# AaronZ345/StyleSinger

Hardware: AMD Instinct MI355X
Metric: mel-frames/sec (end-to-end infer incl. vocoder) (higher is better)
Workload: dtype f32; 1 GPU; c2: batch=8x8.0s utterances per GPU (T=1500 frames, Tp=28, Tr=1500), 100 mel + 2x100 f0 diffusion steps + HiFi-GAN-NSF, exact fp32 MFMA; global_batch=8, frames_per_utterance=1500, parallelism=dp1, diffusion_loops=hipGraph replay, hipgraph_captures=6, frame_bucket=64, mfma_precision=fp32, step_overlap=3 HIP streams: consecutive batches run concurrently

## Files before the change

stylesinger_amd/csrc/wino44_conv.hip:

```cpp
#include "common.h"
#include "device_prims.h"
#include "../../include/stylesinger_hip.h"
#include <type_traits>

namespace {

using namespace ss_dev;

constexpr int BK = 32;
constexpr int LD = BK;
constexpr int BQ = 64;
constexpr int NC = 7;
constexpr int NR = 7;

template <int D>
__device__ __forceinline__ int frame_of_quad(int q) {
  if constexpr (D == 1) return 4 * q;
  else return (q / D) * (4 * D) + (q % D);
}

template <int D, bool LRELU, int BN>
__global__ __launch_bounds__(BN * 4, BN == 64 ? 2 : 1) void wino44_conv_kernel(const ss_conv_gemm_args a, int q_tiles_per_item, int q_tiles,
                                                                               int n_tiles, int groups, int lo_rows) {
  static_assert(BN == 64 || BN == 32, "column tile of 64 or 32");
  constexpr int NT = BN * 4;
  constexpr int RP = NT / 8;
  constexpr int AP = BQ / RP;
  constexpr int BP = BN / RP;
  extern __shared__ __attribute__((aligned(16))) float smem[];
  float* As = smem;
  float* Bs = smem + 2 * BQ * LD;

  const int id = blockIdx.x;
  const int grp = id / (8 * n_tiles);
  const int rem = id % (8 * n_tiles);
  const int qt = grp * 8 + (rem & 7);
  const int nt = rem >> 3;
  if (qt >= q_tiles) return;
  const int b = __builtin_amdgcn_readfirstlane(qt / q_tiles_per_item);
  const int q0 = __builtin_amdgcn_readfirstlane((qt % q_tiles_per_item) * BQ);
  const int n0 = nt * BN;

  const int tid = threadIdx.x, lane = tid & 63, wave = tid >> 6;
  const int wm = BN == 64 ? wave >> 1 : wave, wn = BN == 64 ? wave & 1 : 0;
  const int l31 = lane & 31, lh = lane >> 5;

  const int len = ss_uniform_len(a.lens, b, a.T);
  const int kchunks = a.Kp / BK;
  const int ldw = groups * NC * a.Kp;

  const __amdgpu_buffer_rsrc_t rsrc_a = __builtin_amdgcn_make_buffer_rsrc(
      uniform_ptr(a.A + (int64_t)b * a.a_batch_stride), 0, __builtin_amdgcn_readfirstlane(len * a.lda * 4), 0x00020000);
  const __amdgpu_buffer_rsrc_t rsrc_w =
      __builtin_amdgcn_make_buffer_rsrc(uniform_ptr(a.W), 0, __builtin_amdgcn_readfirstlane(a.Np * ldw * 4), 0x00020000);

  const int st_c4 = tid & 7;
  const int st_row = tid >> 3;
  int roff[AP];
#pragma unroll
  for (int i = 0; i < AP; ++i) roff[i] = ((frame_of_quad<D>(q0 + st_row + i * RP) - lo_rows) * a.lda + st_c4 * 4) * 4;
  const int row_step = D * a.lda * 4;
  const int group_step = 4 * row_step;
  int w_voff[BP];
#pragma unroll
  for (int i = 0; i < BP; ++i) w_voff[i] = ((n0 + st_row + i * RP) * ldw + st_c4 * 4) * 4;

  using Yes = std::true_type;
  using No = std::false_type;
  u32x4 rr[AP][NR], rb[BP];
  auto load_rows = [&](int ci0b, auto ends) {
    ci0b = __builtin_amdgcn_readfirstlane(ci0b);
#pragma unroll
    for (int i = 0; i < AP; ++i)
#pragma unroll
      for (int r = 0; r < NR; ++r)
        if ((r == 0 || r == NR - 1) == decltype(ends)::value) rr[i][r] = __builtin_amdgcn_raw_buffer_load_b128(rsrc_a, roff[i] + r * row_step, ci0b, 0);
  };
  auto load_b = [&](int cb) {
    cb = __builtin_amdgcn_readfirstlane(cb);
#pragma unroll
    for (int i = 0; i < BP; ++i) rb[i] = __builtin_amdgcn_raw_buffer_load_b128(rsrc_w, w_voff[i], cb, 0);
  };
  const float slope = a.a_lrelu;
  auto act_rows = [&]() {
    if constexpr (LRELU) {
#pragma unroll
      for (int i = 0; i < AP; ++i)
#pragma unroll
        for (int r = 0; r < NR; ++r) {
          const f32x4 v = __builtin_bit_cast(f32x4, rr[i][r]);
          const f32x4 sv = v * slope;
          f32x4 o;
          o.x = ss_lrelu_max(v.x, sv.x);
          o.y = ss_lrelu_max(v.y, sv.y);
          o.z = ss_lrelu_max(v.z, sv.z);
          o.w = ss_lrelu_max(v.w, sv.w);
          rr[i][r] = __builtin_bit_cast(u32x4, o);
        }
    }
  };
  int a_wr[AP];
#pragma unroll
  for (int i = 0; i < AP; ++i) a_wr[i] = lds_slot(st_row + i * RP, st_c4);
  float4 tU[AP], tV[AP], tW[AP];
  auto store_a = [&](float* Ad, auto ptag) {
    constexpr int P = decltype(ptag)::value;
#pragma unroll
    for (int i = 0; i < AP; ++i) {
      auto R = [&](int q) { return __builtin_bit_cast(float4, rr[i][q]); };
      float4 v;
      if constexpr (P == 0) {
        tU[i] = vfma(4.f, R(1), vfma(-5.f, R(3), R(5)));
        tV[i] = vfma(4.f, R(0), vfma(-5.f, R(2), R(4)));
        tW[i] = vfma(4.f, R(2), vfma(-5.f, R(4), R(6)));
        v = tU[i];
      } else if constexpr (P == 1) {
        v = vfma(-0.5f, tU[i], tW[i]);
      } else if constexpr (P == 2) {
        v = vfma(-0.5f, tV[i], tU[i]);
      } else if constexpr (P == 3) {
        tV[i] = vfma(2.f, R(1), vfma(-4.f, R(2), vfma(-0.5f, R(3), R(4))));
        tU[i] = vfma(2.f, R(2), vfma(-4.f, R(3), vfma(-0.5f, R(4), R(5))));
        v = vadd(tU[i], tV[i]);
      } else if constexpr (P == 4) {
        v = vsub(tU[i], tV[i]);
      } else if constexpr (P == 5) {
        tV[i] = vfma(0.5f, R(1), vfma(-0.5f, R(3), vsub(R(4), R(2))));
        tU[i] = vfma(0.5f, R(2), vfma(-0.5f, R(4), vsub(R(5), R(3))));
        v = vfma(2.f, tV[i], tU[i]);
      } else {
        v = vfma(-2.f, tV[i], tU[i]);
      }
      *reinterpret_cast<float4*>(Ad + a_wr[i]) = v;
    }
  };
  auto store_b = [&](float* Bd) {
#pragma unroll
    for (int i = 0; i < BP; ++i)
      *reinterpret_cast<float4*>(Bd + lds_slot(st_row + i * RP, st_c4)) = __builtin_bit_cast(float4, rb[i]);
  };

  f32x16 acc[NC];
#pragma unroll
  for (int j = 0; j < NC; ++j)
#pragma unroll
    for (int r = 0; r < 16; ++r) acc[j][r] = 0.f;

  constexpr int ORD[NC] = {5, 6, 0, 1, 2, 3, 4};
  const int kb = a.Kp * 4;
  const int cs = BK * 4;
  const int steps = groups * kchunks;

  const int swz = (l31 >> 1) & 7;
  const int a_row = (wm * 32 + l31) * LD;
  const int b_row = (wn * 32 + l31) * LD;
  auto read_frags = [&](const float* Ac, const float* Bc, int q, float4& af, float4& bf) {
    const int so = ((2 * q + lh) ^ swz) << 2;
    af = *reinterpret_cast<const float4*>(Ac + a_row + so);
    bf = *reinterpret_cast<const float4*>(Bc + b_row + so);
  };
  auto mfma4 = [&](f32x16& c, const float4& af, const float4& bf) {
    c = __builtin_amdgcn_mfma_f32_32x32x2f32(af.x, bf.x, c, 0, 0, 0);
    c = __builtin_amdgcn_mfma_f32_32x32x2f32(af.y, bf.y, c, 0, 0, 0);
    c = __builtin_amdgcn_mfma_f32_32x32x2f32(af.z, bf.z, c, 0, 0, 0);
    c = __builtin_amdgcn_mfma_f32_32x32x2f32(af.w, bf.w, c, 0, 0, 0);
  };
  auto chunk = [&](auto etag, auto ptag, auto stage_tag, auto fetch_b_tag, auto fetch_rows_tag, int wb, int rows_cb, bool new_group) {
    constexpr int P = decltype(ptag)::value;
    constexpr int CUR = (decltype(etag)::value + P) & 1;
    constexpr int PN = (P + 1) % NC;
    const float* Ac = As + CUR * BQ * LD;
    const float* Bc = Bs + CUR * BN * LD;
    float4 af0, af1, bf0, bf1;
    read_frags(Ac, Bc, 0, af0, bf0);
    read_frags(Ac, Bc, 1, af1, bf1);
    __builtin_amdgcn_sched_barrier(0);
    mfma4(acc[ORD[P]], af0, bf0);
    read_frags(Ac, Bc, 2, af0, bf0);
    __builtin_amdgcn_sched_barrier(0);
    mfma4(acc[ORD[P]], af1, bf1);
    read_frags(Ac, Bc, 3, af1, bf1);
    __builtin_amdgcn_sched_barrier(0);
    if constexpr (decltype(stage_tag)::value) {
      if constexpr (PN == 0) act_rows();
      store_a(As + (CUR ^ 1) * BQ * LD, std::integral_constant<int, PN>{});
      store_b(Bs + (CUR ^ 1) * BN * LD);
    }
    __builtin_amdgcn_sched_barrier(0);
    if constexpr (decltype(fetch_b_tag)::value) load_b(wb);
    if constexpr (decltype(fetch_rows_tag)::value) {
      if constexpr (P == 4) {
        if (new_group) {
#pragma unroll
          for (int i = 0; i < AP; ++i) roff[i] += group_step;
        }
        load_rows(rows_cb, No{});
      } else {
        load_rows(rows_cb, Yes{});
      }
    }
    __builtin_amdgcn_sched_barrier(0);
    mfma4(acc[ORD[P]], af0, bf0);
    mfma4(acc[ORD[P]], af1, bf1);
    __syncthreads();
  };
  using P0 = std::integral_constant<int, 0>;
  using P1 = std::integral_constant<int, 1>;
  using P2 = std::integral_constant<int, 2>;
  using P3 = std::integral_constant<int, 3>;
  using P4 = std::integral_constant<int, 4>;
  using P5 = std::integral_constant<int, 5>;
  using P6 = std::integral_constant<int, 6>;

  int g = 0, k = 0;
  auto step = [&](auto etag) {
    const bool wrap = k + 1 == kchunks;
    const int gn = wrap ? g + 1 : g, kn = wrap ? 0 : k + 1;
    const int wcur = g * NC * kb + k * cs, wnext = gn * NC * kb + kn * cs;
    chunk(etag, P0{}, Yes{}, Yes{}, No{}, wcur + ORD[2] * kb, 0, false);
    chunk(etag, P1{}, Yes{}, Yes{}, No{}, wcur + ORD[3] * kb, 0, false);
    chunk(etag, P2{}, Yes{}, Yes{}, No{}, wcur + ORD[4] * kb, 0, false);
    chunk(etag, P3{}, Yes{}, Yes{}, No{}, wcur + ORD[5] * kb, 0, false);
    chunk(etag, P4{}, Yes{}, Yes{}, Yes{}, wcur + ORD[6] * kb, kn * cs, wrap);
    chunk(etag, P5{}, Yes{}, Yes{}, Yes{}, wnext + ORD[0] * kb, kn * cs, false);
    chunk(etag, P6{}, Yes{}, Yes{}, No{}, wnext + ORD[1] * kb, 0, false);
    g = gn;
    k = kn;
  };
  using E0 = std::integral_constant<int, 0>;
  using E1 = std::integral_constant<int, 1>;

  load_rows(0, No{});
  load_rows(0, Yes{});
  load_b(ORD[0] * kb);
  act_rows();
  store_a(As, P0{});
  store_b(Bs);
  load_b(ORD[1] * kb);
  __syncthreads();

  auto last_step = [&](auto etag) {
    const int wcur = g * NC * kb + k * cs;
    chunk(etag, P0{}, Yes{}, Yes{}, No{}, wcur + ORD[2] * kb, 0, false);
    chunk(etag, P1{}, Yes{}, Yes{}, No{}, wcur + ORD[3] * kb, 0, false);
    chunk(etag, P2{}, Yes{}, Yes{}, No{}, wcur + ORD[4] * kb, 0, false);
    chunk(etag, P3{}, Yes{}, Yes{}, No{}, wcur + ORD[5] * kb, 0, false);
    chunk(etag, P4{}, Yes{}, Yes{}, No{}, wcur + ORD[6] * kb, 0, false);
    chunk(etag, P5{}, Yes{}, No{}, No{}, 0, 0, false);
    chunk(etag, P6{}, No{}, No{}, No{}, 0, 0, false);
  };
  if constexpr (BN == 64) {
    for (int s = 0; s + 2 < steps; s += 2) {
      step(E0{});
      step(E1{});
    }
    step(E0{});
    last_step(E1{});
  } else {
    int left = steps;
    for (; left > 2; left -= 2) {
      step(E0{});
      step(E1{});
    }
    if (left == 2) {
      step(E0{});
      last_step(E1{});
    } else {
      last_step(E0{});
    }
  }

  const int col = n0 + wn * 32 + l31;
  const bool col_ok = col < a.N;
  const int oob = col_ok ? 0 : (int)0x80000000;
  const __amdgpu_buffer_rsrc_t rsrc_c = __builtin_amdgcn_make_buffer_rsrc(
      uniform_ptr(a.C + (int64_t)b * a.c_batch_stride), 0, __builtin_amdgcn_readfirstlane((int)((int64_t)a.T * a.ldc * 4)), 0x00020000);
  const __amdgpu_buffer_rsrc_t rsrc_r = __builtin_amdgcn_make_buffer_rsrc(
      uniform_ptr(a.R ? const_cast<float*>(a.R) + (int64_t)b * a.r_batch_stride : a.C), 0,
      __builtin_amdgcn_readfirstlane(a.R ? (int)((int64_t)a.T * a.ldr * 4) : 0), 0x00020000);
  const __amdgpu_buffer_rsrc_t rsrc_p = __builtin_amdgcn_make_buffer_rsrc(
      uniform_ptr(a.C + (int64_t)b * a.c_batch_stride), 0, __builtin_amdgcn_readfirstlane(a.accumulate ? (int)((int64_t)a.T * a.ldc * 4) : 0),
      0x00020000);
  const float bs = (a.bias && col_ok) ? a.bias[col] : 0.f;
  const int row_lim = a.mask_rows ? (len < a.T ? len : a.T) : a.T;
  const int ldc4 = a.ldc * 4, ldr4 = a.ldr * 4;
  const int qbase = q0 + wm * 32 + 4 * lh;
  const bool lrelu_out = a.act == SS_ACT_LRELU_;
#pragma unroll
  for (int rb4 = 0; rb4 < 4; ++rb4) {
    float rv[4][4], pv[4][4];
    int tq[4];
#pragma unroll
    for (int e = 0; e < 4; ++e) {
      tq[e] = frame_of_quad<D>(qbase + e + 8 * rb4);
#pragma unroll
      for (int o = 0; o < 4; ++o) {
        const int t = tq[e] + o * D;
        rv[e][o] = __builtin_bit_cast(float, __builtin_amdgcn_raw_buffer_load_b32(rsrc_r, t * ldr4 + (col * 4 + oob), 0, 0));
        pv[e][o] = __builtin_bit_cast(float, __builtin_amdgcn_raw_buffer_load_b32(rsrc_p, t * ldc4 + (col * 4 + oob), 0, 0));
      }
    }
#pragma unroll
    for (int e = 0; e < 4; ++e) {
      const int r = e + 4 * rb4;
      const float s12 = acc[1][r] + acc[2][r], d12 = acc[1][r] - acc[2][r];
      const float s34 = acc[3][r] + acc[4][r], d34 = acc[3][r] - acc[4][r];
      const float m5 = acc[5][r];
      float z[4];
      z[0] = (acc[0][r] + s12) + (s34 + m5);
      z[1] = fmaf(0.5f, m5, fmaf(2.0f, d34, d12));
      z[2] = fmaf(0.25f, m5, fmaf(4.0f, s34, s12));
      z[3] = fmaf(0.125f, m5, fmaf(8.0f, d34, d12)) + acc[6][r];
#pragma unroll
      for (int o = 0; o < 4; ++o) {
        const int t = tq[e] + o * D;
        float v = (z[o] + bs) * a.pre_scale;
        if (lrelu_out) v = ss_lrelu(v, a.act_slope);
        v = (v + rv[e][o]) * a.post_scale + pv[e][o];
        if (t >= row_lim) v = 0.f;
        __builtin_amdgcn_raw_buffer_store_b32(__builtin_bit_cast(unsigned, v), rsrc_c, t * ldc4 + (col * 4 + oob), 0, 0);
      }
    }
  }
}

template <int D, int BN>
void launch_conv(const ss_conv_gemm_args& a, int k, hipStream_t stream) {
  const int quads_per_item = ss_cdiv(a.T, 4 * D) * D;
  const int q_tiles_per_item = ss_cdiv(quads_per_item, BQ);
  const int q_tiles = q_tiles_per_item * a.B;
  const int n_tiles = a.Np / BN;
  const int grid = ss_cdiv(q_tiles, 8) * 8 * n_tiles;
  const size_t lds = (size_t)2 * (BQ + BN) * LD * sizeof(float);
  const int groups = (k + 3) / 4, lo = (k - 1) / 2 * D;
  auto go = [&](auto kernel) { hipLaunchKernelGGL(kernel, dim3(grid), dim3(BN * 4), lds, stream, a, q_tiles_per_item, q_tiles, n_tiles, groups, lo); };
  if (a.a_lrelu != 1.0f) go(wino44_conv_kernel<D, true, BN>);
  else go(wino44_conv_kernel<D, false, BN>);
}

template <int D>
void launch_conv(const ss_conv_gemm_args& a, int k, hipStream_t stream) {
  if (a.Np % 64 == 0) launch_conv<D, 64>(a, k, stream);
  else launch_conv<D, 32>(a, k, stream);
}

}

extern "C" int ss_wino44_conv_ok(int C, int k, int dilation) {
  const bool fewer = k >= 1 && k <= 11 && (k & 1) && ((k + 3) / 4) * 7 < ((k + 2) / 3) * 6;
  return fewer && C > 0 && C % 32 == 0 && (dilation == 1 || dilation == 3 || dilation == 5) ? 1 : 0;
}

extern "C" int ss_wino44_conv(const ss_conv_gemm_args* args, int k, int dilation, void* stream) {
  SS_CHECK_ARG(args != nullptr, "ss_wino44_conv: null args");
  const ss_conv_gemm_args& a = *args;
  SS_CHECK_ARG(a.A && a.W && a.C, "ss_wino44_conv: null A/W/C");
  SS_CHECK_ARG(a.Cin == a.N && ss_wino44_conv_ok(a.Cin, k, dilation), "ss_wino44_conv: Cin=%d == N=%d (multiple of 32), k=%d (7|11), dilation=%d (1|3|5)",
               a.Cin, a.N, k, dilation);
  SS_CHECK_ARG(a.Kp == a.Cin && a.Np == a.N && (a.lda & 3) == 0 && a.lda >= a.Cin, "ss_wino44_conv: Kp == Cin, Np == N, lda a multiple of 4");
  SS_CHECK_ARG(a.epi == SS_EPI_STORE && (a.act == SS_ACT_NONE_ || a.act == SS_ACT_LRELU_) && !a.a_bias && a.a_scale == 1.0f && !a.mfma_bf16 &&
                   a.group_size == 0,
               "ss_wino44_conv: STORE epilogue, act none|lrelu, no input bias/scale, fp32, one weight set");
  SS_CHECK_ARG(a.a_lrelu > 0.0f && a.a_lrelu <= 1.0f, "ss_wino44_conv: input leaky-relu slope %g must be in (0, 1]", (double)a.a_lrelu);
  SS_CHECK_ARG(((int64_t)a.T + 1024) * a.lda * 4 < (1ll << 31) && (int64_t)a.T * a.ldc * 4 < (1ll << 31) &&
                   (!a.R || (int64_t)a.T * a.ldr * 4 < (1ll << 31)) && (int64_t)a.Np * ((k + 3) / 4) * NC * a.Kp * 4 < (1ll << 31),
               "ss_wino44_conv: item too large for 32-bit offsets");
  if (dilation == 1) launch_conv<1>(a, k, (hipStream_t)stream);
  else if (dilation == 3) launch_conv<3>(a, k, (hipStream_t)stream);
  else launch_conv<5>(a, k, (hipStream_t)stream);
  SS_CHECK_LAUNCH("ss_wino44_conv");
  return SS_OK;
}
```

Measured before the change: 44220 mel-frames/s.

## Reuse Winograd input transforms across tap groups via halo rows in LDS

The Winograd F(4,4)-style conv kernel now stages the transformed input tile once, with extra halo rows (AR=80 rows, four transform slots), and reads shifted rows for each tap group instead of reloading and retransforming the input per group. The number of groups becomes a compile-time template parameter (2 for k=7, 3 for k=11), and the per-chunk schedule is fully unrolled over groups × transform positions, with input fetches spread across sub-steps. This is meant to cut global loads and transform ALU work, at the cost of much more LDS per block and larger, more complex unrolled code that may affect occupancy.

```diff
diff --git a/stylesinger_amd/csrc/wino44_conv.hip b/stylesinger_amd/csrc/wino44_conv.hip
--- a/stylesinger_amd/csrc/wino44_conv.hip
+++ b/stylesinger_amd/csrc/wino44_conv.hip
@@ -12,6 +12,14 @@
 constexpr int BQ = 64;
 constexpr int NC = 7;
 constexpr int NR = 7;
+constexpr int AR = 80;
+constexpr int NA = 4;
+constexpr int SLOT[7] = {0, 1, 2, 0, 1, 2, 3};
+
+__device__ __forceinline__ int formed_here(int x) {
+  asm volatile("" : "+v"(x));
+  return x;
+}
 
 template <int D>
 __device__ __forceinline__ int frame_of_quad(int q) {
@@ -19,17 +27,22 @@
   else return (q / D) * (4 * D) + (q % D);
 }
 
-template <int D, bool LRELU, int BN>
+template <int D, bool LRELU, int BN, int G>
 __global__ __launch_bounds__(BN * 4, BN == 64 ? 2 : 1) void wino44_conv_kernel(const ss_conv_gemm_args a, int q_tiles_per_item, int q_tiles,
-                                                                               int n_tiles, int groups, int lo_rows) {
+                                                                               int n_tiles, int lo_rows) {
   static_assert(BN == 64 || BN == 32, "column tile of 64 or 32");
+  static_assert(G == 2 || G == 3, "two or three tap groups");
   constexpr int NT = BN * 4;
   constexpr int RP = NT / 8;
-  constexpr int AP = BQ / RP;
+  constexpr int MP = BQ / RP;
   constexpr int BP = BN / RP;
+  constexpr int H = (G - 1) * D;
+  constexpr bool HALF = BN == 64;
+  constexpr int AP = HALF ? MP : MP + 1;
+  static_assert(H <= 16 && BQ + 16 <= AR, "halo rows fit one pass and the tile");
   extern __shared__ __attribute__((aligned(16))) float smem[];
   float* As = smem;
-  float* Bs = smem + 2 * BQ * LD;
+  float* Bs = smem + NA * AR * LD;
 
   const int id = blockIdx.x;
   const int grp = id / (8 * n_tiles);
@@ -47,7 +60,7 @@
 
   const int len = ss_uniform_len(a.lens, b, a.T);
   const int kchunks = a.Kp / BK;
-  const int ldw = groups * NC * a.Kp;
+  const int ldw = G * NC * a.Kp;
 
   const __amdgpu_buffer_rsrc_t rsrc_a = __builtin_amdgcn_make_buffer_rsrc(
       uniform_ptr(a.A + (int64_t)b * a.a_batch_stride), 0, __builtin_amdgcn_readfirstlane(len * a.lda * 4), 0x00020000);
@@ -56,11 +69,16 @@
 
   const int st_c4 = tid & 7;
   const int st_row = tid >> 3;
+  constexpr int NOROW = (int)0x80000000;
   int roff[AP];
 #pragma unroll
-  for (int i = 0; i < AP; ++i) roff[i] = ((frame_of_quad<D>(q0 + st_row + i * RP) - lo_rows) * a.lda + st_c4 * 4) * 4;
+  for (int i = 0; i < AP; ++i) {
+    const int row = st_row + i * RP;
+    roff[i] = row < BQ + H ? ((frame_of_quad<D>(q0 + row) - lo_rows) * a.lda + st_c4 * 4) * 4 : NOROW;
+  }
+  const int h_row = BQ + (tid >> 4), h_c2 = tid & 15;
+  const int hoff = h_row < BQ + H ? ((frame_of_quad<D>(q0 + h_row) - lo_rows) * a.lda + h_c2 * 2) * 4 : NOROW;
   const int row_step = D * a.lda * 4;
-  const int group_step = 4 * row_step;
   int w_voff[BP];
 #pragma unroll
   for (int i = 0; i < BP; ++i) w_voff[i] = ((n0 + st_row + i * RP) * ldw + st_c4 * 4) * 4;
@@ -68,77 +86,94 @@
   using Yes = std::true_type;
   using No = std::false_type;
   u32x4 rr[AP][NR], rb[BP];
-  auto load_rows = [&](int ci0b, auto ends) {
-    ci0b = __builtin_amdgcn_readfirstlane(ci0b);
-#pragma unroll
-    for (int i = 0; i < AP; ++i)
-#pragma unroll
-      for (int r = 0; r < NR; ++r)
-        if ((r == 0 || r == NR - 1) == decltype(ends)::value) rr[i][r] = __builtin_amdgcn_raw_buffer_load_b128(rsrc_a, roff[i] + r * row_step, ci0b, 0);
+  u32x2 rh[NR];
+  auto load_rows = [&](int i, int cb, auto ends) {
+    const int o = formed_here(roff[i]);
+#pragma unroll
+    for (int r = 0; r < NR; ++r)
+      if ((r == 0 || r == NR - 1) == decltype(ends)::value) rr[i][r] = __builtin_amdgcn_raw_buffer_load_b128(rsrc_a, o + r * row_step, cb, 0);
+  };
+  auto load_half = [&](int cb, auto ends) {
+    const int o = formed_here(hoff);
+#pragma unroll
+    for (int r = 0; r < NR; ++r)
+      if ((r == 0 || r == NR - 1) == decltype(ends)::value) rh[r] = __builtin_amdgcn_raw_buffer_load_b64(rsrc_a, o + r * row_step, cb, 0);
   };
   auto load_b = [&](int cb) {
-    cb = __builtin_amdgcn_readfirstlane(cb);
 #pragma unroll
     for (int i = 0; i < BP; ++i) rb[i] = __builtin_amdgcn_raw_buffer_load_b128(rsrc_w, w_voff[i], cb, 0);
   };
   const float slope = a.a_lrelu;
-  auto act_rows = [&]() {
+  auto act_rows = [&](int i) {
     if constexpr (LRELU) {
 #pragma unroll
-      for (int i = 0; i < AP; ++i)
-#pragma unroll
-        for (int r = 0; r < NR; ++r) {
-          const f32x4 v = __builtin_bit_cast(f32x4, rr[i][r]);
-          const f32x4 sv = v * slope;
-          f32x4 o;
-          o.x = ss_lrelu_max(v.x, sv.x);
-          o.y = ss_lrelu_max(v.y, sv.y);
-          o.z = ss_lrelu_max(v.z, sv.z);
-          o.w = ss_lrelu_max(v.w, sv.w);
-          rr[i][r] = __builtin_bit_cast(u32x4, o);
-        }
+      for (int r = 0; r < NR; ++r) {
+        const f32x4 v = __builtin_bit_cast(f32x4, rr[i][r]);
+        const f32x4 sv = v * slope;
+        f32x4 o;
+        o.x = ss_lrelu_max(v.x, sv.x);
+        o.y = ss_lrelu_max(v.y, sv.y);
+        o.z = ss_lrelu_max(v.z, sv.z);
+        o.w = ss_lrelu_max(v.w, sv.w);
+        rr[i][r] = __builtin_bit_cast(u32x4, o);
+      }
+    }
+  };
+  auto act_half = [&]() {
+    if constexpr (LRELU) {
+#pragma unroll
+      for (int r = 0; r < NR; ++r) {
+        const f32x2 v = __builtin_bit_cast(f32x2, rh[r]);
+        const f32x2 sv = v * slope;
+        f32x2 o;
+        o.x = ss_lrelu_max(v.x, sv.x);
+        o.y = ss_lrelu_max(v.y, sv.y);
+        rh[r] = __builtin_bit_cast(u32x2, o);
+      }
     }
   };
   int a_wr[AP];
 #pragma unroll
   for (int i = 0; i < AP; ++i) a_wr[i] = lds_slot(st_row + i * RP, st_c4);
-  float4 tU[AP], tV[AP], tW[AP];
-  auto store_a = [&](float* Ad, auto ptag) {
-    constexpr int P = decltype(ptag)::value;
-#pragma unroll
-    for (int i = 0; i < AP; ++i) {
-      auto R = [&](int q) { return __builtin_bit_cast(float4, rr[i][q]); };
-      float4 v;
-      if constexpr (P == 0) {
-        tU[i] = vfma(4.f, R(1), vfma(-5.f, R(3), R(5)));
-        tV[i] = vfma(4.f, R(0), vfma(-5.f, R(2), R(4)));
-        tW[i] = vfma(4.f, R(2), vfma(-5.f, R(4), R(6)));
-        v = tU[i];
-      } else if constexpr (P == 1) {
-        v = vfma(-0.5f, tU[i], tW[i]);
-      } else if constexpr (P == 2) {
-        v = vfma(-0.5f, tV[i], tU[i]);
-      } else if constexpr (P == 3) {
-        tV[i] = vfma(2.f, R(1), vfma(-4.f, R(2), vfma(-0.5f, R(3), R(4))));
-        tU[i] = vfma(2.f, R(2), vfma(-4.f, R(3), vfma(-0.5f, R(4), R(5))));
-        v = vadd(tU[i], tV[i]);
-      } else if constexpr (P == 4) {
-        v = vsub(tU[i], tV[i]);
-      } else if constexpr (P == 5) {
-        tV[i] = vfma(0.5f, R(1), vfma(-0.5f, R(3), vsub(R(4), R(2))));
-        tU[i] = vfma(0.5f, R(2), vfma(-0.5f, R(4), vsub(R(5), R(3))));
-        v = vfma(2.f, tV[i], tU[i]);
-      } else {
-        v = vfma(-2.f, tV[i], tU[i]);
-      }
-      *reinterpret_cast<float4*>(Ad + a_wr[i]) = v;
-    }
+  const int h_wr = lds_slot(h_row, h_c2 >> 1) + 2 * (h_c2 & 1);
+  auto build = [&](auto settag, auto R, float* Ad, int w) {
+    constexpr int SET = decltype(settag)::value;
+    using V = decltype(R(0));
+    auto put = [&](int pos, const V& v) { *reinterpret_cast<V*>(Ad + SLOT[pos] * AR * LD + w) = v; };
+    if constexpr (SET == 0) {
+      const V c5 = vfma(4.f, R(1), vfma(-5.f, R(3), R(5)));
+      const V F0 = vfma(4.f, R(0), vfma(-5.f, R(2), R(4)));
+      const V E2 = vfma(4.f, R(2), vfma(-5.f, R(4), R(6)));
+      put(0, c5);
+      put(1, vfma(-0.5f, c5, E2));
+      put(2, vfma(-0.5f, F0, c5));
+    } else if constexpr (SET == 1) {
+      const V Pv = vfma(2.f, R(1), vfma(-4.f, R(2), vfma(-0.5f, R(3), R(4))));
+      const V Pu = vfma(2.f, R(2), vfma(-4.f, R(3), vfma(-0.5f, R(4), R(5))));
+      put(3, vadd(Pu, Pv));
+      put(4, vsub(Pu, Pv));
+    } else {
+      const V Qv = vfma(0.5f, R(1), vfma(-0.5f, R(3), vsub(R(4), R(2))));
+      const V Qu = vfma(0.5f, R(2), vfma(-0.5f, R(4), vsub(R(5), R(3))));
+      put(5, vfma(2.f, Qv, Qu));
+      put(6, vfma(-2.f, Qv, Qu));
+    }
+  };
+  auto store_a = [&](int i, auto settag) {
+    build(settag, [&](int q) { return __builtin_bit_cast(float4, rr[i][q]); }, As, a_wr[i]);
+  };
+  auto store_half = [&](auto settag) {
+    build(settag, [&](int q) { return __builtin_bit_cast(float2, rh[q]); }, As, h_wr);
   };
   auto store_b = [&](float* Bd) {
 #pragma unroll
     for (int i = 0; i < BP; ++i)
       *reinterpret_cast<float4*>(Bd + lds_slot(st_row + i * RP, st_c4)) = __builtin_bit_cast(float4, rb[i]);
   };
+  constexpr int HALO_G = G - 1;
+  auto pass_group = [](int i) constexpr { return i >= MP ? HALO_G : i / (MP / 2); };
+  auto fetch_mid_at = [](int pg) constexpr { return 4 * G + pg; };
+  auto fetch_ends_at = [](int pg) constexpr { return 6 * G + pg - 1; };
 
   f32x16 acc[NC];
 #pragma unroll
@@ -149,54 +184,74 @@
   constexpr int ORD[NC] = {5, 6, 0, 1, 2, 3, 4};
   const int kb = a.Kp * 4;
   const int cs = BK * 4;
-  const int steps = groups * kchunks;
-
-  const int swz = (l31 >> 1) & 7;
-  const int a_row = (wm * 32 + l31) * LD;
-  const int b_row = (wn * 32 + l31) * LD;
-  auto read_frags = [&](const float* Ac, const float* Bc, int q, float4& af, float4& bf) {
-    const int so = ((2 * q + lh) ^ swz) << 2;
-    af = *reinterpret_cast<const float4*>(Ac + a_row + so);
-    bf = *reinterpret_cast<const float4*>(Bc + b_row + so);
-  };
+  constexpr int NS = NC * G;
+
+  auto slot0 = [&](int row) { return (row * LD + ((lh ^ ((row >> 1) & 7)) << 2)) * 4; };
+  int a_s0[G];
+#pragma unroll
+  for (int g = 0; g < G; ++g) a_s0[g] = slot0(wm * 32 + l31 + g * D);
+  const int b_s0 = slot0(wn * 32 + l31);
   auto mfma4 = [&](f32x16& c, const float4& af, const float4& bf) {
     c = __builtin_amdgcn_mfma_f32_32x32x2f32(af.x, bf.x, c, 0, 0, 0);
     c = __builtin_amdgcn_mfma_f32_32x32x2f32(af.y, bf.y, c, 0, 0, 0);
     c = __builtin_amdgcn_mfma_f32_32x32x2f32(af.z, bf.z, c, 0, 0, 0);
     c = __builtin_amdgcn_mfma_f32_32x32x2f32(af.w, bf.w, c, 0, 0, 0);
   };
-  auto chunk = [&](auto etag, auto ptag, auto stage_tag, auto fetch_b_tag, auto fetch_rows_tag, int wb, int rows_cb, bool new_group) {
-    constexpr int P = decltype(ptag)::value;
-    constexpr int CUR = (decltype(etag)::value + P) & 1;
-    constexpr int PN = (P + 1) % NC;
-    const float* Ac = As + CUR * BQ * LD;
-    const float* Bc = Bs + CUR * BN * LD;
+  auto sub = [&](auto etag, auto stag, int k, bool more) {
+    constexpr int E = decltype(etag)::value, S = decltype(stag)::value;
+    constexpr int P = S / G, GI = S % G;
+    constexpr int BCUR = (E * G + S) & 1;
+    constexpr int SET = P == 6 ? 0 : P == 2 ? 1 : P == 4 ? 2 : -1;
+    const float* Ac = As + SLOT[P] * AR * LD;
+    const float* Bc = Bs + BCUR * BN * LD;
+    const int a_s = a_s0[GI], b_s = b_s0;
+    auto read_frags = [&](int q, float4& af, float4& bf) {
+      af = *reinterpret_cast<const float4*>(reinterpret_cast<const char*>(Ac) + (a_s ^ (32 * q)));
+      bf = *reinterpret_cast<const float4*>(reinterpret_cast<const char*>(Bc) + (b_s ^ (32 * q)));
+    };
     float4 af0, af1, bf0, bf1;
-    read_frags(Ac, Bc, 0, af0, bf0);
-    read_frags(Ac, Bc, 1, af1, bf1);
+    read_frags(0, af0, bf0);
+    read_frags(1, af1, bf1);
     __builtin_amdgcn_sched_barrier(0);
     mfma4(acc[ORD[P]], af0, bf0);
-    read_frags(Ac, Bc, 2, af0, bf0);
+    read_frags(2, af0, bf0);
     __builtin_amdgcn_sched_barrier(0);
     mfma4(acc[ORD[P]], af1, bf1);
-    read_frags(Ac, Bc, 3, af1, bf1);
+    read_frags(3, af1, bf1);
     __builtin_amdgcn_sched_barrier(0);
-    if constexpr (decltype(stage_tag)::value) {
-      if constexpr (PN == 0) act_rows();
-      store_a(As + (CUR ^ 1) * BQ * LD, std::integral_constant<int, PN>{});
-      store_b(Bs + (CUR ^ 1) * BN * LD);
-    }
+    if constexpr (SET >= 0) {
+      if (SET != 0 || more) {
+        using Set = std::integral_constant<int, SET>;
+#pragma unroll
+        for (int i = 0; i < AP; ++i)
+          if (pass_group(i) == GI) {
+            if constexpr (SET == 0) act_rows(i);
+            store_a(i, Set{});
+          }
+        if constexpr (HALF && HALO_G == GI) {
+          if constexpr (SET == 0) act_half();
+          store_half(Set{});
+        }
+      }
+    }
+    if (S + 1 < NS || more) store_b(Bs + (BCUR ^ 1) * BN * LD);
     __builtin_amdgcn_sched_barrier(0);
-    if constexpr (decltype(fetch_b_tag)::value) load_b(wb);
-    if constexpr (decltype(fetch_rows_tag)::value) {
-      if constexpr (P == 4) {
-        if (new_group) {
-#pragma unroll
-          for (int i = 0; i < AP; ++i) roff[i] += group_step;
+    {
+      constexpr int S2 = (S + 2) % NS;
+      constexpr int wo = (S2 % G) * NC + ORD[S2 / G];
+      if constexpr (S + 2 < NS) load_b(__builtin_amdgcn_readfirstlane(wo * kb + k * cs));
+      else if (more) load_b(__builtin_amdgcn_readfirstlane(wo * kb + (k + 1) * cs));
+    }
+    if constexpr (P >= 4) {
+      if (more) {
+        const int cb = __builtin_amdgcn_readfirstlane((k + 1) * cs);
+#pragma unroll
+        for (int i = 0; i < AP; ++i) {
+          if (fetch_mid_at(pass_group(i)) == S) load_rows(i, cb, No{});
+          if (fetch_ends_at(pass_group(i)) == S) load_rows(i, cb, Yes{});
         }
-        load_rows(rows_cb, No{});
-      } else {
-        load_rows(rows_cb, Yes{});
+        if constexpr (HALF && fetch_mid_at(HALO_G) == S) load_half(cb, No{});
+        if constexpr (HALF && fetch_ends_at(HALO_G) == S) load_half(cb, Yes{});
       }
     }
     __builtin_amdgcn_sched_barrier(0);
@@ -204,69 +259,42 @@
     mfma4(acc[ORD[P]], af1, bf1);
     __syncthreads();
   };
-  using P0 = std::integral_constant<int, 0>;
-  using P1 = std::integral_constant<int, 1>;
-  using P2 = std::integral_constant<int, 2>;
-  using P3 = std::integral_constant<int, 3>;
-  using P4 = std::integral_constant<int, 4>;
-  using P5 = std::integral_constant<int, 5>;
-  using P6 = std::integral_constant<int, 6>;
-
-  int g = 0, k = 0;
-  auto step = [&](auto etag) {
-    const bool wrap = k + 1 == kchunks;
-    const int gn = wrap ? g + 1 : g, kn = wrap ? 0 : k + 1;
-    const int wcur = g * NC * kb + k * cs, wnext = gn * NC * kb + kn * cs;
-    chunk(etag, P0{}, Yes{}, Yes{}, No{}, wcur + ORD[2] * kb, 0, false);
-    chunk(etag, P1{}, Yes{}, Yes{}, No{}, wcur + ORD[3] * kb, 0, false);
-    chunk(etag, P2{}, Yes{}, Yes{}, No{}, wcur + ORD[4] * kb, 0, false);
-    chunk(etag, P3{}, Yes{}, Yes{}, No{}, wcur + ORD[5] * kb, 0, false);
-    chunk(etag, P4{}, Yes{}, Yes{}, Yes{}, wcur + ORD[6] * kb, kn * cs, wrap);
-    chunk(etag, P5{}, Yes{}, Yes{}, Yes{}, wnext + ORD[0] * kb, kn * cs, false);
-    chunk(etag, P6{}, Yes{}, Yes{}, No{}, wnext + ORD[1] * kb, 0, false);
-    g = gn;
-    k = kn;
-  };
+  using Set0 = std::integral_constant<int, 0>;
   using E0 = std::integral_constant<int, 0>;
   using E1 = std::integral_constant<int, 1>;
 
-  load_rows(0, No{});
-  load_rows(0, Yes{});
+#pragma unroll
+  for (int i = 0; i < AP; ++i) {
+    load_rows(i, 0, No{});
+    load_rows(i, 0, Yes{});
+  }
+  if constexpr (HALF) {
+    load_half(0, No{});
+    load_half(0, Yes{});
+  }
   load_b(ORD[0] * kb);
-  act_rows();
-  store_a(As, P0{});
+#pragma unroll
+  for (int i = 0; i < AP; ++i) {
+    act_rows(i);
+    store_a(i, Set0{});
+  }
+  if constexpr (HALF) {
+    act_half();
+    store_half(Set0{});
+  }
   store_b(Bs);
-  load_b(ORD[1] * kb);
+  load_b(__builtin_amdgcn_readfirstlane((NC + ORD[0]) * kb));
   __syncthreads();
 
-  auto last_step = [&](auto etag) {
-    const int wcur = g * NC * kb + k * cs;
-    chunk(etag, P0{}, Yes{}, Yes{}, No{}, wcur + ORD[2] * kb, 0, false);
-    chunk(etag, P1{}, Yes{}, Yes{}, No{}, wcur + ORD[3] * kb, 0, false);
-    chunk(etag, P2{}, Yes{}, Yes{}, No{}, wcur + ORD[4] * kb, 0, false);
-    chunk(etag, P3{}, Yes{}, Yes{}, No{}, wcur + ORD[5] * kb, 0, false);
-    chunk(etag, P4{}, Yes{}, Yes{}, No{}, wcur + ORD[6] * kb, 0, false);
-    chunk(etag, P5{}, Yes{}, No{}, No{}, 0, 0, false);
-    chunk(etag, P6{}, No{}, No{}, No{}, 0, 0, false);
-  };
-  if constexpr (BN == 64) {
-    for (int s = 0; s + 2 < steps; s += 2) {
-      step(E0{});
-      step(E1{});
-    }
-    step(E0{});
-    last_step(E1{});
+  auto chunk = [&](auto etag, int k, bool more) {
+    unrolled_steps([&](auto stag) { sub(etag, stag, k, more); }, std::make_integer_sequence<int, NS>{});
+  };
+  if constexpr (G == 2) {
+    for (int k = 0; k < kchunks; ++k) chunk(E0{}, k, k + 1 < kchunks);
   } else {
-    int left = steps;
-    for (; left > 2; left -= 2) {
-      step(E0{});
-      step(E1{});
-    }
-    if (left == 2) {
-      step(E0{});
-      last_step(E1{});
-    } else {
-      last_step(E0{});
+    for (int k = 0; k < kchunks; k += 2) {
+      chunk(E0{}, k, k + 1 < kchunks);
+      if (BN == 64 || k + 1 < kchunks) chunk(E1{}, k + 1, k + 2 < kchunks);
     }
   }
 
@@ -324,24 +352,25 @@
   }
 }
 
-template <int D, int BN>
-void launch_conv(const ss_conv_gemm_args& a, int k, hipStream_t stream) {
+template <int D, int BN, int G>
+void launch_conv(const ss_conv_gemm_args& a, hipStream_t stream) {
   const int quads_per_item = ss_cdiv(a.T, 4 * D) * D;
   const int q_tiles_per_item = ss_cdiv(quads_per_item, BQ);
   const int q_tiles = q_tiles_per_item * a.B;
   const int n_tiles = a.Np / BN;
   const int grid = ss_cdiv(q_tiles, 8) * 8 * n_tiles;
-  const size_t lds = (size_t)2 * (BQ + BN) * LD * sizeof(float);
-  const int groups = (k + 3) / 4, lo = (k - 1) / 2 * D;
-  auto go = [&](auto kernel) { hipLaunchKernelGGL(kernel, dim3(grid), dim3(BN * 4), lds, stream, a, q_tiles_per_item, q_tiles, n_tiles, groups, lo); };
-  if (a.a_lrelu != 1.0f) go(wino44_conv_kernel<D, true, BN>);
-  else go(wino44_conv_kernel<D, false, BN>);
+  const size_t lds = (size_t)(NA * AR + 2 * BN) * LD * sizeof(float);
+  const int lo = (4 * G - 2) / 2 * D;
+  auto go = [&](auto kernel) { hipLaunchKernelGGL(kernel, dim3(grid), dim3(BN * 4), lds, stream, a, q_tiles_per_item, q_tiles, n_tiles, lo); };
+  if (a.a_lrelu != 1.0f) go(wino44_conv_kernel<D, true, BN, G>);
+  else go(wino44_conv_kernel<D, false, BN, G>);
 }
 
 template <int D>
 void launch_conv(const ss_conv_gemm_args& a, int k, hipStream_t stream) {
-  if (a.Np % 64 == 0) launch_conv<D, 64>(a, k, stream);
-  else launch_conv<D, 32>(a, k, stream);
+  const bool wide = a.Np % 64 == 0;
+  if (k == 7) wide ? launch_conv<D, 64, 2>(a, stream) : launch_conv<D, 32, 2>(a, stream);
+  else wide ? launch_conv<D, 64, 3>(a, stream) : launch_conv<D, 32, 3>(a, stream);
 }
 
 }
```

Result: faster. 44730 mel-frames/s, median of 6 (+1.2%).
